# aifoundry-org/MHAQ

Hardware: AMD Instinct MI355X
Metric: qat_images_per_sec (higher is better)
Workload: dtype f32; 1 GPU; ResNet-18 ImageNet-1k QAT step, AEWGS weights per-channel + STE activations, Sym-KL distillation from FP teacher, RAdam, synthetic 224x224, channels_last memory format; per_gpu_batch=250, global_batch=250, parallelism=dp1, sync_batchnorm=False, weight_backward_groups=3, cudnn_benchmark=False

## Files before the change

### include/mhaq_fq.h

```cpp
#ifndef MHAQ_FQ_H
#define MHAQ_FQ_H

#include <stddef.h>
#include <stdint.h>

#ifdef __cplusplus
extern "C" {
#endif

#define MHAQ_FQ_ABI_VERSION 4

enum { MHAQ_FQ_STE = 0, MHAQ_FQ_EWGS = 1, MHAQ_FQ_AEWGS = 2, MHAQ_FQ_LSQ = 3 };

enum {
  MHAQ_FQ_EINVAL = -1,
  MHAQ_FQ_EWORKSPACE = -2,
  MHAQ_FQ_EALIGN = -3,
  MHAQ_FQ_EUNSUPPORTED = -4
};

enum {
  MHAQ_FQ_FLAG_BELOW_MIN = 1,
  MHAQ_FQ_FLAG_ABOVE_MAX = 2,
  MHAQ_FQ_FLAG_NOT_INTEGER = 4
// ... 20 lines not shown
                   void* workspace, size_t workspace_bytes, void* stream);

int mhaq_fq_pt_bwd_partials(const float* x, const float* g, float* gx, int64_t n,
                            const float* s, const float* zp, const float* lo, const float* hi,
                            int method, const float* col_stats, int64_t period,
                            const int8_t* r_sign, uint64_t seed, uint64_t offset, const uint64_t* offset_dev, int count_ties,
                            void* workspace, size_t workspace_bytes, int32_t* nparts_out, void* stream);
int mhaq_fq_pt_bwd_finalize(const void* workspace, int32_t nparts, float* grads , void* stream);

int mhaq_fq_act_fwd(const float* x, float* y, int64_t n,
                    const float* log_act_s, const float* log_act_q, const float* act_b,
                    float* params_out , float* qstats, int32_t* flags,
                    void* workspace, size_t workspace_bytes, void* stream);
size_t mhaq_fq_act_bwd_workspace_bytes(int64_t n);
int mhaq_fq_act_bwd(const float* x, const float* g, float* gx, int64_t n, const float* params ,
                    int method, const int8_t* r_sign, uint64_t seed, uint64_t offset, const uint64_t* offset_dev,
                    float* grads , void* workspace, size_t workspace_bytes, void* stream);

typedef struct {
  const float* partials;
  int64_t nparts;
} mhaq_act_finalize_desc;
int mhaq_fq_act_bwd_partials(const float* x, const float* g, float* gx, int64_t n, const float* params ,
                             int method, const int8_t* r_sign, uint64_t seed, uint64_t offset,
                             const uint64_t* offset_dev, void* workspace, size_t workspace_bytes,
                             int32_t* nparts_out, void* stream);
int mhaq_fq_act_bwd_finalize_multi(const mhaq_act_finalize_desc* descs_device, int nquant,
                                   float* grads_out , void* stream);

enum { MHAQ_FQ_DT_BF16 = 1, MHAQ_FQ_DT_F16 = 2 };
int mhaq_fq_act_fwd_x16(const void* x, void* y, int64_t n, int dtype,
                        const float* log_act_s, const float* log_act_q, const float* act_b,
                        float* params_out , float* qstats, int32_t* flags,
                        void* workspace, size_t workspace_bytes, void* stream);
int mhaq_fq_act_bwd_x16(const void* x, const void* g, void* gx, int64_t n, int dtype, const float* params ,
                        int method, const int8_t* r_sign, uint64_t seed, uint64_t offset, const uint64_t* offset_dev,
                        float* grads , void* workspace, size_t workspace_bytes, void* stream);
int mhaq_fq_act_bwd_partials_x16(const void* x, const void* g, void* gx, int64_t n, int dtype,
                                 const float* params , int method, const int8_t* r_sign, uint64_t seed,
                                 uint64_t offset, const uint64_t* offset_dev, void* workspace, size_t workspace_bytes,
                                 int32_t* nparts_out, void* stream);

int mhaq_fq_act_relu_fwd(const float* z, const float* addend, float* y, float* a_out, int64_t n,
                         const float* log_act_s, const float* log_act_q, const float* act_b,
                         float* params_out , void* stream);
int mhaq_fq_act_relu_bwd(const float* z, const float* g_y, const float* g_a, float* gx, int64_t n,
                         const float* params , int method, uint64_t seed, uint64_t offset,
                         const uint64_t* offset_dev, float* grads , void* workspace, size_t workspace_bytes,
                         void* stream);
int mhaq_fq_act_relu_bwd_partials(const float* z, const float* g_y, const float* g_a, float* gx, int64_t n,
                                  const float* params , int method, uint64_t seed, uint64_t offset,
                                  const uint64_t* offset_dev, void* workspace, size_t workspace_bytes,
                                  int32_t* nparts_out, void* stream);

size_t mhaq_fq_minmax_workspace_bytes(int64_t n);
int mhaq_fq_minmax(const float* x, int64_t n, float* out ,
                   void* workspace, size_t workspace_bytes, void* stream);

int mhaq_fq_row_minmax(const float* w, int64_t co, int64_t row, float* mn_out ,
                       float* mx_out , void* stream);

int mhaq_fq_pt_tie_scatter(const float* w, float* gw, int64_t n, const float* zp,
                           const float* grads , void* stream);

size_t mhaq_fq_pt_aewgs_colstats_workspace_bytes(int64_t co, int64_t row);
int mhaq_fq_pt_aewgs_colstats(const float* w, const float* G, int64_t co, int64_t row,
                              const float* s, const float* zp, const float* lo, const float* hi,
                              float* stats, void* workspace, size_t workspace_bytes, void* stream);

int mhaq_fq_pc_fwd(const float* w, float* wq, float* zp_out , float* q_out ,
                   const float* s , int64_t co, int64_t row, void* stream);

int mhaq_fq_pc_bwd(const float* w, const float* G, float* gw, float* g_s ,
                   const float* s , const float* zp ,
                   int64_t co, int64_t row, int method, const float* stats,
                   const float* gzp_extra ,
                   const int8_t* r_sign, uint64_t seed, uint64_t offset, const uint64_t* offset_dev, void* stream);

int mhaq_fq_wlayer_fwd(const float* w, float* wq, const float* log_s , int64_t co, int64_t row,
                       float* s_out, float* zp_out, float* mx_out, float* lwq_out ,
                       void* stream);
int mhaq_fq_wlayer_bwd(const float* w, const float* G, float* gw, float* g_log_s ,
                       const float* s, const float* zp, const float* mx, const float* g_lwq ,
                       int64_t co, int64_t row, int method, const float* stats,
                       const float* gzp_extra, const int8_t* r_sign, uint64_t seed, uint64_t offset, const uint64_t* offset_dev,
                       void* stream);

int64_t mhaq_fq_wlayer_pt_max_elements(void);
int mhaq_fq_wlayer_pt_fwd(const float* w, float* wq, const float* log_s , int64_t n,
                          float* aux , void* stream);
int mhaq_fq_wlayer_pt_bwd(const float* w, const float* G, float* gw, float* g_log_s ,
                          const float* aux, const float* g_lwq, int64_t n, int method,
                          const int8_t* r_sign, uint64_t seed, uint64_t offset, const uint64_t* offset_dev, void* stream);

size_t mhaq_fq_wlayer_ptl_workspace_bytes(int64_t n);
int mhaq_fq_wlayer_ptl_fwd(const float* w, float* wq, const float* log_s , int64_t n, float* aux ,
                           void* workspace, size_t workspace_bytes, void* stream);
int mhaq_fq_wlayer_ptl_bwd(const float* w, const float* G, float* gw, float* g_log_s ,
                           const float* aux , const float* g_lwq , int64_t n, int method,
                           const float* col_stats, int64_t period,
                           const int8_t* r_sign, uint64_t seed, uint64_t offset, const uint64_t* offset_dev,
                           void* workspace, size_t workspace_bytes, void* stream);

typedef struct {
  const float* w;
  const float* log_s;
// ... 58 lines not shown
```

### mhaq_amd/_lib.py

```python
from __future__ import annotations

import ctypes as C
import os
import re

_HERE = os.path.dirname(os.path.abspath(__file__))
LIB_PATH = os.environ.get("MHAQ_FQ_LIB") or os.path.join(_HERE, "csrc", "libmhaq_fq.so")
HEADER_PATH = os.path.join(os.path.dirname(_HERE), "include", "mhaq_fq.h")

_p = C.c_void_p
_i64 = C.c_int64
_u64 = C.c_uint64
_sz = C.c_size_t
_int = C.c_int

DT_BF16 = 1
DT_F16 = 2

SIGNATURES = {
    "mhaq_fq_abi_version": (_int, []),
    "mhaq_fq_error_string": (C.c_char_p, [_int]),
    "mhaq_fq_fill_r": (_int, [_p, _i64, _u64, _u64, _p]),
    "mhaq_fq_pt_fwd_workspace_bytes": (_sz, [_i64]),
    "mhaq_fq_pt_fwd": (_int, [_p, _p, _i64, _p, _p, _p, _p, _p, _p, _p, _p, _sz, _p]),
    "mhaq_fq_pt_bwd_workspace_bytes": (_sz, [_i64]),
    "mhaq_fq_pt_bwd": (_int, [_p, _p, _p, _i64, _p, _p, _p, _p, _int, _p, _i64, _p, _u64, _u64, _p, _int, _p, _p, _sz, _p]),
    "mhaq_fq_pt_bwd_partials": (_int, [_p, _p, _p, _i64, _p, _p, _p, _p, _int, _p, _i64, _p, _u64, _u64, _p, _int, _p, _sz,
                                       _p, _p]),
    "mhaq_fq_pt_bwd_finalize": (_int, [_p, C.c_int32, _p, _p]),
    "mhaq_fq_act_fwd": (_int, [_p, _p, _i64, _p, _p, _p, _p, _p, _p, _p, _sz, _p]),
    "mhaq_fq_act_bwd_workspace_bytes": (_sz, [_i64]),
    "mhaq_fq_act_bwd": (_int, [_p, _p, _p, _i64, _p, _int, _p, _u64, _u64, _p, _p, _p, _sz, _p]),
    "mhaq_fq_act_bwd_partials": (_int, [_p, _p, _p, _i64, _p, _int, _p, _u64, _u64, _p, _p, _sz, _p, _p]),
    "mhaq_fq_act_bwd_finalize_multi": (_int, [_p, _int, _p, _p]),
    "mhaq_fq_act_fwd_x16": (_int, [_p, _p, _i64, _int, _p, _p, _p, _p, _p, _p, _p, _sz, _p]),
    "mhaq_fq_act_bwd_x16": (_int, [_p, _p, _p, _i64, _int, _p, _int, _p, _u64, _u64, _p, _p, _p, _sz, _p]),
    "mhaq_fq_act_bwd_partials_x16": (_int, [_p, _p, _p, _i64, _int, _p, _int, _p, _u64, _u64, _p, _p, _sz, _p, _p]),
    "mhaq_fq_act_relu_fwd": (_int, [_p, _p, _p, _p, _i64, _p, _p, _p, _p, _p]),
    "mhaq_fq_act_relu_bwd": (_int, [_p, _p, _p, _p, _i64, _p, _int, _u64, _u64, _p, _p, _p, _sz, _p]),
    "mhaq_fq_act_relu_bwd_partials": (_int, [_p, _p, _p, _p, _i64, _p, _int, _u64, _u64, _p, _p, _sz, _p, _p]),
    "mhaq_fq_minmax_workspace_bytes": (_sz, [_i64]),
    "mhaq_fq_minmax": (_int, [_p, _i64, _p, _p, _sz, _p]),
    "mhaq_fq_row_minmax": (_int, [_p, _i64, _i64, _p, _p, _p]),
    "mhaq_fq_pt_tie_scatter": (_int, [_p, _p, _i64, _p, _p, _p]),
    "mhaq_fq_pt_aewgs_colstats_workspace_bytes": (C.c_size_t, [_i64, _i64]),
    "mhaq_fq_pt_aewgs_colstats": (_int, [_p, _p, _i64, _i64, _p, _p, _p, _p, _p, _p, C.c_size_t, _p]),
    "mhaq_fq_pc_fwd": (_int, [_p, _p, _p, _p, _p, _i64, _i64, _p]),
    "mhaq_fq_pc_bwd": (_int, [_p, _p, _p, _p, _p, _p, _i64, _i64, _int, _p, _p, _p, _u64, _u64, _p, _p]),
    "mhaq_fq_pc_aewgs_stats": (_int, [_p, _p, _p, _p, _i64, _i64, _p, _p]),
    "mhaq_fq_wlayer_fwd": (_int, [_p, _p, _p, _i64, _i64, _p, _p, _p, _p, _p]),
    "mhaq_fq_wlayer_bwd": (_int, [_p, _p, _p, _p, _p, _p, _p, _p, _i64, _i64, _int, _p, _p, _p, _u64, _u64, _p, _p]),
    "mhaq_fq_wlayer_fwd_multi": (_int, [_p, _int, _i64, _i64, _p, _p, _p]),
    "mhaq_fq_wlayer_bwd_multi": (_int, [_p, _int, _i64, _i64, _p, _p, _p, _int, _p, _u64, _u64, _p, _p]),
    "mhaq_fq_wlayer_bwd_group": (_int, [_p, _int, _i64, _i64, _p, _i64, _p, _p, _int, _p, _u64, _u64, _p, _p]),
    "mhaq_fq_wlayer_aewgs_stats_group": (_int, [_p, _int, _i64, _p, _i64, _p, _p]),
    "mhaq_fq_pc_quantize": (_int, [_p, _p, _p, _p, _p, _i64, _i64, _p, _p]),
    "mhaq_fq_wlayer_pt_max_elements": (_i64, []),
    "mhaq_fq_wlayer_pt_fwd": (_int, [_p, _p, _p, _i64, _p, _p]),
    "mhaq_fq_wlayer_pt_bwd": (_int, [_p, _p, _p, _p, _p, _p, _i64, _int, _p, _u64, _u64, _p, _p]),
    "mhaq_fq_wlayer_ptl_workspace_bytes": (_sz, [_i64]),
    "mhaq_fq_wlayer_ptl_fwd": (_int, [_p, _p, _p, _i64, _p, _p, _sz, _p]),
    "mhaq_fq_wlayer_ptl_bwd": (_int, [_p, _p, _p, _p, _p, _p, _i64, _int, _p, _i64, _p, _u64, _u64, _p, _p, _sz, _p]),
    "mhaq_fq_vec_fwd": (_int, [_p, _p, _p, _p, _p, _i64, _p]),
    "mhaq_fq_vec_aewgs_stats": (_int, [_p, _p, _p, _p, _i64, _p, _p]),
    "mhaq_fq_vec_bwd": (_int, [_p, _p, _p, _p, _p, _p, _p, _i64, _int, _p, _p, _u64, _u64, _p, _p]),
    "mhaq_fq_potential_loss_fwd": (_int, [_p, _p, _p, _i64, _p, _p, _i64, C.c_float, C.c_float, C.c_float, _int,
                                          _p, _int, _p, _p]),
    "mhaq_fq_potential_loss_bwd": (_int, [_p, _p, _p, _p, _i64, _p, _p, _i64, C.c_float, C.c_float, C.c_float,
                                          _p, _p, _p, _p, _p, _p]),
    "mhaq_fq_noise_fwd": (_int, [_p, _p, _i64, _p]),
    "mhaq_fq_noise_bwd_workspace_bytes": (_sz, [_i64, _i64]),
    "mhaq_fq_noise_bwd": (_int, [_p, _p, _p, _p, _i64, _i64, _int, _p, _i64, _p, _u64, _u64, _p, _p, _sz, _p]),
}

_lib = None


class MhaqFqError(RuntimeError):
    pass


def header_functions():
    with open(HEADER_PATH) as f:
        src = re.sub(r"/\*.*?\*/", "", f.read(), flags=re.S)
    return sorted(set(re.findall(r"\b(mhaq_fq_\w+)\s*\(", src)))


def _try_build() -> None:
    import fcntl
    import subprocess
    import sys
    csrc = os.path.dirname(LIB_PATH)
    with open(os.path.join(csrc, ".build.lock"), "w") as lock:
# ... 37 lines not shown
```

### mhaq_amd/csrc/torch_binding.cpp

```cpp
#include <torch/extension.h>
#include <torch/version.h>
#include <torch/csrc/autograd/custom_function.h>

#include <c10/hip/HIPCachingAllocator.h>
#include <c10/hip/HIPGraphsC10Utils.h>
#include <c10/hip/HIPStream.h>
#include <c10/core/DeviceGuard.h>
#include <dlfcn.h>

#include <algorithm>
#include <atomic>
#include <chrono>
#include <cstring>
#include <map>
#include <memory>
#include <mutex>
#include <string>
#include <unordered_map>
#include <vector>

#include "../../include/mhaq_fq.h"

namespace py = pybind11;
using at::Tensor;
using torch::autograd::AutogradContext;
using torch::autograd::variable_list;

namespace {

#define MHAQ_API(X)                                                                                                   \
  X(mhaq_fq_abi_version) X(mhaq_fq_error_string) X(mhaq_fq_act_fwd) X(mhaq_fq_act_bwd_workspace_bytes)                \
  X(mhaq_fq_act_bwd) X(mhaq_fq_act_bwd_partials) X(mhaq_fq_act_bwd_finalize_multi) X(mhaq_fq_wlayer_fwd)              \
  X(mhaq_fq_wlayer_bwd) X(mhaq_fq_pc_aewgs_stats) X(mhaq_fq_wlayer_fwd_multi) X(mhaq_fq_wlayer_bwd_group)             \
  X(mhaq_fq_wlayer_aewgs_stats_group) X(mhaq_fq_wlayer_pt_fwd) X(mhaq_fq_wlayer_pt_bwd)                               \
  X(mhaq_fq_potential_loss_fwd) X(mhaq_fq_potential_loss_bwd) X(mhaq_fq_wlayer_ptl_workspace_bytes)                   \
  X(mhaq_fq_wlayer_ptl_fwd) X(mhaq_fq_wlayer_ptl_bwd) X(mhaq_fq_pt_aewgs_colstats_workspace_bytes)                     \
  X(mhaq_fq_pt_aewgs_colstats) X(mhaq_fq_act_fwd_x16) X(mhaq_fq_act_bwd_x16) X(mhaq_fq_act_bwd_partials_x16)                    \
  X(mhaq_fq_act_relu_fwd) X(mhaq_fq_act_relu_bwd) X(mhaq_fq_act_relu_bwd_partials)

struct Api {
#define X(n) decltype(&::n) n = nullptr;
  MHAQ_API(X)
#undef X
  void* handle = nullptr;
  std::string path;
};
Api A;

struct MhaqError : std::runtime_error {
  using std::runtime_error::runtime_error;
};

void bind_library(const std::string& path) {
  if (A.handle && A.path == path) return;
  void* h = dlopen(path.c_str(), RTLD_NOW | RTLD_LOCAL);
  if (!h) throw MhaqError("cannot load " + path + ": " + dlerror() + " (there is no CPU fallback)");
  Api a;
#define X(n)                                                                        \
  a.n = reinterpret_cast<decltype(a.n)>(dlsym(h, #n));                              \
  if (!a.n) throw MhaqError(std::string(#n) + " is not exported by " + path);
  MHAQ_API(X)
#undef X
  if (a.mhaq_fq_abi_version() != MHAQ_FQ_ABI_VERSION) throw MhaqError("libmhaq_fq.so ABI version mismatch");
  a.handle = h;
  a.path = path;
  A = a;
}

inline void need_lib() {
  if (!A.handle) throw MhaqError("the C-ABI library is not bound (mhaq_amd._ext.bind)");
}

inline void check(int rc, const char* what) {
  if (rc != 0)
    throw MhaqError(std::string(what) + " failed: " + A.mhaq_fq_error_string(rc) + " (code " + std::to_string(rc) + ")");
}

inline void* cur_stream(const Tensor& t) {
  return (void*)c10::hip::getCurrentHIPStream(t.device().index()).stream();
}

inline bool capturing() {
  return c10::hip::currentStreamCaptureStatusMayInitCtx() != c10::hip::CaptureStatus::None;
}

#define MHAQ_ON_DEVICE_OF(t) const c10::OptionalDeviceGuard mhaq_device_guard_(at::device_of(t))

inline const float* fptr(const Tensor& t) { return static_cast<const float*>(t.const_data_ptr()); }
inline float* fptr_mut(const Tensor& t) { return static_cast<float*>(t.mutable_data_ptr()); }
inline const float* fptr_or_null(const Tensor& t) { return t.defined() ? fptr(t) : nullptr; }

// ... 422 lines not shown
    const int64_t t0 = now_ns();
    auto saved = ctx->get_saved_variables();
    const std::vector<int64_t> ic = ctx->saved_data["i"].toIntVector();
    variable_list out(10);
    const bool g_y_def = grads[0].defined(), g_a_def = ic[4]  != 0 && grads.size() > 2 && grads[2].defined();
    if (!g_y_def && !g_a_def) return out;
    const int64_t t1 = now_ns();
    const size_t e = ic[5] != 0 ? 1 : 0;
    ActGrads res = act_backward(ctx, t0, t1, saved, ic, grads[0], g_a_def ? grads[2] : Tensor(), false,
                                1 + e,
                               [](const ActBwdLaunch& a) {
      if (a.hub)
        check(A.mhaq_fq_act_relu_bwd_partials(fptr(a.x), fptr(a.g), fptr_or_null(a.ga), fptr_mut(a.gx), a.n, fptr(a.params),
                                              a.method, a.d.seed, a.d.offset, a.d.offset_dev, a.ws, a.nb, a.nparts,
                                              a.stream),
              "mhaq_fq_act_relu_bwd_partials");
      else
        check(A.mhaq_fq_act_relu_bwd(fptr(a.x), fptr(a.g), fptr_or_null(a.ga), fptr_mut(a.gx), a.n, fptr(a.params), a.method,
                                     a.d.seed, a.d.offset, a.d.offset_dev, a.gr, a.ws, a.nb, a.stream),
              "mhaq_fq_act_relu_bwd");
    });
    if (e && ctx->needs_input_grad(1)) out[1] = res.gx;
    if (ctx->needs_input_grad(0)) out[0] = std::move(res.gx);
    for (int c = 0; c < 3; ++c) out[2 + c] = std::move(res.gp[c]);
    return out;
  }
};

std::tuple<Tensor, std::optional<Tensor>, Tensor, Tensor, Tensor> act_relu_layer(
    const Tensor& z, const std::optional<Tensor>& addend, const Tensor& log_s, const Tensor& log_q, const Tensor& b,
    int64_t method, bool want_act, int64_t hub_id, int64_t slot, int64_t rank) {
  need_lib();
  MHAQ_ON_DEVICE_OF(z);
  TORCH_CHECK(z.is_cuda() && z.scalar_type() == at::kFloat && z.is_non_overlapping_and_dense(),
              "act_relu_layer: z must be a dense float32 device tensor");
  const bool has_add = addend.has_value() && addend->defined();
  TORCH_CHECK(!has_add || (addend->device() == z.device() && addend->scalar_type() == at::kFloat &&
                           addend->sizes() == z.sizes() && addend->strides() == z.strides()),
              "act_relu_layer: addend must have z's device, dtype, shape and strides");
  TORCH_CHECK(!has_add || want_act, "act_relu_layer: with an addend the ReLU output is an output of the op (want_act)");
  TORCH_CHECK(method == MHAQ_FQ_STE || method == MHAQ_FQ_LSQ || method == MHAQ_FQ_EWGS,
              "act_relu_layer: STE, LSQ or EWGS");
  check_act_params("act_relu_layer", log_s, log_q, b);
  const int64_t t0 = now_ns();
  auto out = ActReluFn::apply(z, addend, log_s, log_q, b, method, want_act, hub_id, slot, rank);
  const Tensor& params = out[1];
  std::tuple<Tensor, std::optional<Tensor>, Tensor, Tensor, Tensor> res{
      out[0], want_act ? std::optional<Tensor>(out[2]) : std::nullopt, params, params.narrow(0, 0, 1),
      params.narrow(0, 3, 1)};
  tick(T_ACT_FWD, t0, now_ns());
  return res;
}

struct Pre {
  bool has = false;
  Tensor wq, s, zp, mx, lwq;
};

PyObject* g_allreduce_avg = nullptr;
std::atomic<bool> g_dist_active{false};

void allreduce_avg(const Tensor& t) {
  py::gil_scoped_acquire gil;
  if (!g_allreduce_avg) throw MhaqError("AEWGS statistics exchange requested but no all-reduce is installed");
  py::reinterpret_borrow<py::object>(g_allreduce_avg)(t);
}

class WeightLayerFn : public torch::autograd::Function<WeightLayerFn> {
 public:
  static variable_list forward(AutogradContext* ctx, const Tensor& w, const Tensor& log_s, int64_t method,
                               const std::optional<Tensor>& r_sign, bool zp_grad, const Pre& pre, int64_t rank,
                               bool distributed) {
    const int64_t co = w.size(0), row = co ? w.numel() / co : 0;
    Tensor wq, s, zp, mx, lwq;
    if (pre.has) {
      wq = pre.wq; s = pre.s; zp = pre.zp; mx = pre.mx; lwq = pre.lwq;
    } else {
      wq = at::empty_like(w);
      Tensor aux = at::empty({4, co}, w.options());
      s = aux.select(0, 0); zp = aux.select(0, 1); mx = aux.select(0, 2); lwq = aux.select(0, 3);
      check(A.mhaq_fq_wlayer_fwd(fptr(w), fptr_mut(wq), fptr(log_s), co, row, fptr_mut(s), fptr_mut(zp), fptr_mut(mx),
                                 fptr_mut(lwq), cur_stream(w)),
            "mhaq_fq_wlayer_fwd");
    }
    weight_save_ctx(ctx, {w, s, zp, mx}, r_sign, method, rank, log_s);
    ctx->saved_data["dist"] = distributed;
    if (!zp_grad) ctx->mark_non_differentiable({s, zp});
    return {wq, zp, s, lwq};
  }

  static variable_list backward(AutogradContext* ctx, variable_list grads) {
    auto saved = ctx->get_saved_variables();
    const Tensor &w = saved[0], &s = saved[1], &zp = saved[2], &mx = saved[3];
    const bool has_r = saved.size() > 4;
    const int64_t method = ctx->saved_data["method"].toInt();
    Tensor G = grads[0].defined() ? like_layout(grads[0], w) : at::zeros_like(w);
    Tensor gzp_extra = grads[1].defined() ? grads[1].contiguous() : Tensor();
    Tensor g_lwq = grads[3].defined() ? grads[3].contiguous() : Tensor();
    const int64_t co = w.size(0), row = co ? w.numel() / co : 0;
    Tensor stats;
    if (method == MHAQ_FQ_AEWGS && ctx->saved_data["dist"].toBool()) {
      stats = at::empty({3, co}, w.options());
      check(A.mhaq_fq_pc_aewgs_stats(fptr(w), fptr(G), fptr(s), fptr(zp), co, row, fptr_mut(stats), cur_stream(w)),
            "mhaq_fq_pc_aewgs_stats");
      allreduce_avg(stats);
    }
// ... 514 lines not shown
    return d;
  }, py::arg("reset") = true);
  m.def("bound_library", []() { return A.path; });

  m.def("rng_manual_seed", [](uint64_t seed) { std::lock_guard<std::mutex> g(R.mu); R.seed = seed; R.seeded = true; R.count = 0; });
  m.def("rng_seed", []() -> py::object { std::lock_guard<std::mutex> g(R.mu); return R.seeded ? py::object(py::int_(R.seed)) : py::none(); });
  m.def("rng_next", [](int64_t rank) {
    std::lock_guard<std::mutex> g(R.mu);
    if (!R.seeded) throw MhaqError("sign stream used before it was seeded");
    return std::make_pair(R.seed ^ ((uint64_t)rank * kGolden), ++R.count);
  });
  m.def("rng_drawn", []() { std::lock_guard<std::mutex> g(R.mu); return R.count; });
  m.def("rng_set_drawn", [](uint64_t n) { std::lock_guard<std::mutex> g(R.mu); R.count = n; });
  m.def("rng_set_base", [](const std::optional<Tensor>& base) {
    std::lock_guard<std::mutex> g(R.mu);
    R.base = (base.has_value() && base->defined()) ? *base : Tensor();
  });
  m.def("rng_base", []() -> std::optional<Tensor> {
    std::lock_guard<std::mutex> g(R.mu);
    return R.base.defined() ? std::optional<Tensor>(R.base) : std::nullopt;
  });

  m.def("set_allreduce_avg", [](py::object fn) {
    g_allreduce_avg = fn.is_none() ? nullptr : fn.inc_ref().ptr();
  });
  m.def("set_dist_active", [](bool v) { g_dist_active.store(v); });

  m.def("hub_create", &hub_create);
  m.def("hub_destroy", [](int64_t id) { g_hubs.erase(id); });
  m.def("hub_begin", &hub_begin);
  m.def("hub_clear_pending", [](int64_t id) { auto h = g_hubs.get(id); std::lock_guard<std::mutex> g(h->mu); h->pending.clear(); });
  m.def("hub_release_captured", [](int64_t id) { g_hubs.get(id)->release_captured(); });
  m.def("hub_state", [](int64_t id) {
    auto h = g_hubs.get(id);
    std::lock_guard<std::mutex> g(h->mu);
    py::dict d;
    d["tables"] = h->tables.entries.size();
    d["captured_tables"] = h->tables.captured();
    d["retired"] = h->retired.size();
    d["pending"] = h->pending.size();
    d["has_table"] = h->last_table.defined();
    int64_t bytes = 0;
    for (auto& w : h->ws) if (w.defined()) bytes += w.numel();
    for (auto& w : h->retired) bytes += w.numel();
    d["workspace_bytes"] = bytes;
    return d;
  });
  m.def("act_layer", &act_layer, py::arg("x"), py::arg("log_act_s"), py::arg("log_act_q"), py::arg("act_b"),
        py::arg("method"), py::arg("r_sign") = py::none(), py::arg("hub") = 0, py::arg("slot") = 0, py::arg("rank") = 0);
  m.def("act_relu_layer", &act_relu_layer, py::arg("z"), py::arg("addend"), py::arg("log_act_s"), py::arg("log_act_q"),
        py::arg("act_b"), py::arg("method"), py::arg("want_act"), py::arg("hub") = 0, py::arg("slot") = 0,
        py::arg("rank") = 0);

  m.def("weight_layer", &weight_layer, py::arg("w"), py::arg("log_wght_s"), py::arg("method"),
        py::arg("r_sign") = py::none(), py::arg("zp_grad") = false, py::arg("pre") = py::none(), py::arg("rank") = 0);
  m.def("weight_layer_pt", &weight_layer_pt, py::arg("w"), py::arg("log_wght_s"), py::arg("method"),
        py::arg("r_sign") = py::none(), py::arg("rank") = 0);
  m.def("weight_layer_ptl", &weight_layer_ptl, py::arg("w"), py::arg("log_wght_s"), py::arg("method"),
        py::arg("r_sign") = py::none(), py::arg("rank") = 0);

  m.def("plan_create", &plan_create);
  m.def("plan_destroy", [](int64_t id) { g_plans.erase(id); });
  m.def("plan_forward", &plan_forward);
  m.def("plan_group_apply", &plan_group_apply);
  m.def("plan_release_captured", [](int64_t id) {
    auto p = g_plans.get(id);
    std::lock_guard<std::mutex> g(p->mu);
    for (auto& grp : p->groups) if (grp.pool) grp.pool->release_captured();
    p->fwd_tables.release_captured();
  });
  m.def("plan_state", [](int64_t id) {
    auto p = g_plans.get(id);
    std::lock_guard<std::mutex> g(p->mu);
    py::dict d;
    d["fwd_tables"] = p->fwd_tables.entries.size();
    py::list pools;
    for (auto& grp : p->groups) {
      py::dict e;
      size_t used = 0, held = 0, size = 0;
      if (grp.pool) {
        size = grp.pool->keys.size();
        for (size_t i = 0; i < size; ++i) { used += grp.pool->used[i]; held += grp.pool->held[i]; }
      }
      e["size"] = size; e["used"] = used; e["held"] = held;
      pools.append(e);
    }
    d["pools"] = pools;
    return d;
  });

  m.def("potential_loss", &potential_loss);
}
```

### mhaq_amd/qat.py

```python
from __future__ import annotations

import contextlib
import copy
import time
from dataclasses import dataclass, field
from typing import Optional

import torch
import torch.distributed as dist
from torch import nn

from . import ops
from ._lib import MhaqFqError
from .enums import QNMethod, QScheme
from .loss import FusedPotentialLoss, FusedPotentialLossNoPred, SymmetricalKL
from .wrap import get_model_values, quantize_model


@dataclass
class QATConfig:
    qscheme: QScheme = QScheme.PER_CHANNEL
    qnmethod: QNMethod = QNMethod.AEWGS
    act_bit: int = 1
    weight_bit: int = 1
    calib_act_bit: int = 10
    calib_weight_bit: int = 10
    excluded_layers: tuple = ("conv1", "fc")
    quantize_bias: bool = False
    distillation: bool = True
    learning_rate: float = 3e-4
    warmup: int = 100
    scale_lr: float = 1.0
    scale_t: float = 2.0
    sync_batchnorm: bool = True
    overlap_teacher: bool = True
    joint_act_finalize: bool = True
    student_high_priority: bool = False
    multi_weight_forward: bool = True
    weight_backward_group_elems: int = 4 << 20
    fuse_blocks: bool = True
    criterion: nn.Module = field(default_factory=nn.CrossEntropyLoss)
    autocast_dtype: Optional[torch.dtype] = None


@torch.no_grad()
def calibrate_weights(model: nn.Module, wbits: int, max_bits: int = 24, row_minmax_fn=None) -> None:
    row_minmax_fn = row_minmax_fn or ops.row_minmax
    for m in model.modules():
        if hasattr(m, "log_wght_s") and hasattr(m, "weight"):
            mn, mx = row_minmax_fn(m.weight)
            mn, mx = mn.cpu(), mx.cpu()
            if m.log_wght_s.numel() == 1 and mn.numel() != 1:
                mn, mx = mn.min(), mx.max()
            if not m.log_wght_s.requires_grad:
                wbits = max_bits
            floor = torch.log2((mx - mn) / (2 ** wbits - 1)).reshape(m.log_wght_s.shape)
            m.log_wght_s.copy_(torch.max(m.log_wght_s.detach().cpu(), floor))


def _cpu_row_minmax(w):
    dims = tuple(range(1, w.dim()))
    return w.detach().amin(dims), w.detach().amax(dims)


@torch.no_grad()
def calibrate_activations(model: nn.Module, batches, abits: int, max_bits: int = 24, minmax_fn=None) -> None:
    minmax_fn = minmax_fn or ops.minmax
    acts = [m for m in model.modules() if hasattr(m, "log_act_s") and hasattr(m, "act_b")]
    seen = {id(a): [] for a in acts}
    hooks = [a.register_forward_pre_hook(lambda mod, inp: seen[id(mod)].append(minmax_fn(inp[0]))) for a in acts]
    was_training = model.training
    model.eval()
    for x in batches:
        model(x)
    for h in hooks:
        h.remove()
    model.train(was_training)
    for a in acts:
        mm = torch.stack(seen[id(a)]).cpu()
        mn, mx = mm[:, 0].min(), mm[:, 1].max()
        if not a.log_act_q.requires_grad and not a.log_act_s.requires_grad:
            abits = max_bits
        if mx - mn > 0:
            log_s = torch.log2((mx - mn) / (2 ** abits - 1))
            a.act_b.fill_(mn)
            a.log_act_s.fill_(log_s)
            a.log_act_q.fill_(log_s + abits)
        else:
            a.log_act_q.zero_(), a.log_act_s.zero_(), a.act_b.fill_(mn)
            a.log_act_q.requires_grad_(False), a.log_act_s.requires_grad_(False), a.act_b.requires_grad_(False)


class TemperatureSchedule:
# ... 23 lines not shown
        new_lr = self.lr * self.lr_t if past else self.lr * self.total_batch / self.warmup
        self._set_lr(optimizer, new_lr)
        return new_lr


class _QATModule(nn.Module):

    def __init__(self, net, qscheme, act_hub=None, weight_forward=None):
        super().__init__()
        self.model = net
        self.qscheme = qscheme
        self.act_hub = act_hub
        self.weight_forward = weight_forward
        self._quantized = None

    def forward(self, x):
        if self.weight_forward is not None and self.training:
            self.weight_forward.run()
        if self.act_hub is not None and self.training:
            self.act_hub.begin()
        if self._quantized is None:
            self._quantized = [m for m in self.model.modules() if hasattr(m, "log_wght_s") or hasattr(m, "log_act_s")]
        try:
            return (self.model(x), *get_model_values(self.model, self.qscheme, modules=self._quantized))
        finally:
            if self.act_hub is not None:
                self.act_hub.end()


class QATTrainer:
    def __init__(self, net: nn.Module, cfg: QATConfig, device, calib_batches=None, layers=None,
                 distributed=None, minmax_fn=None, optimizer_factory=None,
                 multi_tensor_weights=False, capture_graph=None, loss_classes=None):
        self.cfg, self.device = cfg, torch.device(device)
        if cfg.autocast_dtype is not None and cfg.autocast_dtype != torch.bfloat16:
            raise ValueError(f"QATConfig.autocast_dtype: {cfg.autocast_dtype} is not supported (None or torch.bfloat16; "
                             "float16 training needs loss scaling, which this trainer does not do)")
        self.distributed = ops._dist_active() if distributed is None else distributed
        net = net.to(self.device)
        self.teacher = copy.deepcopy(net).eval().requires_grad_(False) if cfg.distillation else None
        quantize_model(net, cfg.qscheme, cfg.qnmethod, cfg.excluded_layers, cfg.quantize_bias, cfg.act_bit,
                       layers=layers)
        net.to(self.device)
        if calib_batches is not None:
            calibrate_weights(net, cfg.calib_weight_bit,
                              row_minmax_fn=_cpu_row_minmax if self.device.type != "cuda" else None)
            calibrate_activations(net, calib_batches, cfg.calib_act_bit, minmax_fn=minmax_fn)
        if self.distributed and cfg.sync_batchnorm and self.device.type == "cuda":
            net = nn.SyncBatchNorm.convert_sync_batchnorm(net)
        if cfg.fuse_blocks and layers is None and self.device.type == "cuda":
            from . import fused_blocks
            if fused_blocks.enabled_by_env():
                fused_blocks.install(net)
        self.net = net
        self.teacher_stream = None
        if cfg.distillation and cfg.overlap_teacher and self.device.type == "cuda":
            self.teacher_stream = torch.cuda.Stream(device=self.device)
        self._hp_stream = None
        if cfg.student_high_priority and self.device.type == "cuda":
            self._hp_stream = torch.cuda.Stream(device=self.device, priority=-1)
        self.multi = None
        if multi_tensor_weights and self.distributed:
            raise ValueError("multi_tensor_weights is a single-GPU option (the data-parallel trainer keeps the "
                             "per-layer ops: AEWGS statistics all-reduce + gradient overlap)")
        if multi_tensor_weights:
            from .multi import MultiTensorWeightQuant
            self.multi = MultiTensorWeightQuant(net)
        self.act_hub = None
        if cfg.joint_act_finalize and self.device.type == "cuda" and (layers is None):
            from .act_hub import ActGradHub
            hub = ActGradHub(net)
            self.act_hub = hub if len(hub) > 1 else None
        self.weight_forward = None
        if cfg.multi_weight_forward and self.multi is None and self.device.type == "cuda" and layers is None:
            from .multi import MultiTensorWeightQuant
            try:
                wf = MultiTensorWeightQuant(net, joint_backward=False,
                                            backward_group_elems=cfg.weight_backward_group_elems)
                self.weight_forward = wf if wf.nlayers > 1 else None
            except ValueError:
                pass
        self.module = _QATModule(net, cfg.qscheme, self.act_hub, self.weight_forward)
        self._flat_sync = False
        want_capture = capture_graph
        if want_capture is None:
            want_capture = "auto" if (layers is None and optimizer_factory is None and not multi_tensor_weights) else False
        if self.distributed and want_capture and self.device.type == "cuda" and self.multi is None:
            step_collectives = any(isinstance(m, nn.SyncBatchNorm) for m in net.modules()) or any(
                ops._method_value(m.Q.qnmethod) == QNMethod.AEWGS.value for m in net.modules() if hasattr(m, "Q")
            ) or next(iter(net.buffers()), None) is not None
            self._flat_sync = not step_collectives
        if self.distributed:
            for p in [m.log_b_s for m in net.modules() if hasattr(m, "log_b_s")]:
                p.requires_grad_(False)
            if self._flat_sync:
                with torch.no_grad():
                    for t in list(net.parameters()) + list(net.buffers()):
                        dist.broadcast(t, 0)
            else:
                self._wrap_ddp()
        if loss_classes is None:
            if self.device.type != "cuda":
                raise MhaqFqError("QATTrainer on a CPU device needs loss_classes (and layers): the fake-quant path and "
                                  "its PotentialLoss run only as HIP kernels (no CPU fallback by design)")
            loss_classes = (FusedPotentialLoss, FusedPotentialLossNoPred)
        if cfg.distillation:
# ... 279 lines not shown
```

Before: 6119 images/s.

## Add custom HIP BatchNorm backward kernels for channels-last fp32 student BN layers

Swaps the student's nn.BatchNorm2d modules for a subclass whose autograd node keeps the framework forward but runs a custom HIP backward. The backward does a chunked fp64 per-channel reduction, a finalize kernel that writes dweight/dbias and per-channel constants, and a vectorized dx kernel with non-temporal loads and stores for large tensors. The aim is to replace MIOpen/PyTorch BN backward on channels-last fp32 inputs. It costs three launches per BN plus a workspace allocation, and it falls back to the stock backward when the inputs are not eligible.

```diff
diff --git a/include/mhaq_fq.h b/include/mhaq_fq.h
--- a/include/mhaq_fq.h
+++ b/include/mhaq_fq.h
@@ -96,6 +96,11 @@
                                   const float* params , int method, uint64_t seed, uint64_t offset,
                                   const uint64_t* offset_dev, void* workspace, size_t workspace_bytes,
                                   int32_t* nparts_out, void* stream);
+
+size_t mhaq_fq_bn_bwd_workspace_bytes(int64_t m, int64_t c);
+int mhaq_fq_bn_bwd(const float* x, const float* dy, const float* mean, const float* invstd, const float* weight,
+                   float* dx, float* dweight, float* dbias, int64_t m, int64_t c,
+                   void* workspace, size_t workspace_bytes, void* stream);
 
 size_t mhaq_fq_minmax_workspace_bytes(int64_t n);
 int mhaq_fq_minmax(const float* x, int64_t n, float* out ,
diff --git a/mhaq_amd/_lib.py b/mhaq_amd/_lib.py
--- a/mhaq_amd/_lib.py
+++ b/mhaq_amd/_lib.py
@@ -39,6 +39,8 @@
     "mhaq_fq_act_relu_fwd": (_int, [_p, _p, _p, _p, _i64, _p, _p, _p, _p, _p]),
     "mhaq_fq_act_relu_bwd": (_int, [_p, _p, _p, _p, _i64, _p, _int, _u64, _u64, _p, _p, _p, _sz, _p]),
     "mhaq_fq_act_relu_bwd_partials": (_int, [_p, _p, _p, _p, _i64, _p, _int, _u64, _u64, _p, _p, _sz, _p, _p]),
+    "mhaq_fq_bn_bwd_workspace_bytes": (_sz, [_i64, _i64]),
+    "mhaq_fq_bn_bwd": (_int, [_p, _p, _p, _p, _p, _p, _p, _p, _i64, _i64, _p, _sz, _p]),
     "mhaq_fq_minmax_workspace_bytes": (_sz, [_i64]),
     "mhaq_fq_minmax": (_int, [_p, _i64, _p, _p, _sz, _p]),
     "mhaq_fq_row_minmax": (_int, [_p, _i64, _i64, _p, _p, _p]),
diff --git a/mhaq_amd/bn_backward.py b/mhaq_amd/bn_backward.py
--- /dev/null
+++ b/mhaq_amd/bn_backward.py
@@ -0,0 +1,46 @@
+from __future__ import annotations
+
+import os
+
+import torch
+from torch import nn
+
+ENV_SWITCH = "MHAQ_BN_BACKWARD"
+
+
+def enabled_by_env() -> bool:
+    return os.environ.get(ENV_SWITCH, "1").strip().lower() not in ("0", "false", "off", "no")
+
+
+class HipBackwardBatchNorm2d(nn.BatchNorm2d):
+
+    def forward(self, input):
+        if (not self.training or not self.track_running_stats or not self.affine or not input.is_cuda
+                or input.dtype != torch.float32 or self.weight.dtype != torch.float32):
+            return super().forward(input)
+        self._check_input_dim(input)
+        exponential_average_factor = 0.0 if self.momentum is None else self.momentum
+        if self.num_batches_tracked is not None:
+            self.num_batches_tracked.add_(1)
+            if self.momentum is None:
+                exponential_average_factor = 1.0 / float(self.num_batches_tracked)
+            else:
+                exponential_average_factor = self.momentum
+        from . import _ext
+        return _ext.ext().bn_train(input, self.weight, self.bias, self.running_mean, self.running_var,
+                                   exponential_average_factor, self.eps, torch.backends.cudnn.enabled)
+
+
+def install(model: nn.Module) -> int:
+    switched = 0
+    for m in model.modules():
+        if type(m) is nn.BatchNorm2d:
+            m.__class__ = HipBackwardBatchNorm2d
+            switched += 1
+    return switched
+
+
+def uninstall(model: nn.Module) -> None:
+    for m in model.modules():
+        if type(m) is HipBackwardBatchNorm2d:
+            m.__class__ = nn.BatchNorm2d
diff --git a/mhaq_amd/csrc/bn_bwd.hip b/mhaq_amd/csrc/bn_bwd.hip
--- /dev/null
+++ b/mhaq_amd/csrc/bn_bwd.hip
@@ -0,0 +1,236 @@
+#include "fq_common.hpp"
+
+namespace mhaq {
+
+template <bool NT>
+__device__ __forceinline__ vf4 bn_ld4(const float* p, int64_t vidx) {
+  const vf4* q = reinterpret_cast<const vf4*>(p) + vidx;
+  return NT ? __builtin_nontemporal_load(q) : *q;
+}
+__device__ __forceinline__ void bn_st4(float* p, int64_t vidx, vf4 v) {
+  __builtin_nontemporal_store(v, reinterpret_cast<vf4*>(p) + vidx);
+}
+
+constexpr int kBnCols = 16;
+constexpr int kBnRedU = 4;
+constexpr int kBnMinRows = 448;
+constexpr int kBnMaxChunks = 2048;
+constexpr int kBnDxU = 2;
+constexpr int64_t kBnMaxChannels = 1ll << 22;
+constexpr int kBnNConst = 5;
+
+struct BnGeom {
+  int64_t rows;
+  int64_t nchunks;
+  int ncol;
+};
+static inline BnGeom bn_geom(int64_t m, int64_t c) {
+  const int64_t cv = c >> 2;
+  const int64_t cols = cv < kBnCols ? cv : kBnCols;
+  const int64_t rpp = kBlock / cols;
+  const int64_t unit = rpp * kBnRedU;
+  int64_t rows = (m + kBnMaxChunks - 1) / kBnMaxChunks;
+  if (rows < kBnMinRows) rows = kBnMinRows;
+  rows = (rows + unit - 1) / unit * unit;
+  BnGeom g;
+  g.rows = rows;
+  g.nchunks = (m + rows - 1) / rows;
+  g.ncol = (int)((cv + kBnCols - 1) / kBnCols);
+  return g;
+}
+
+constexpr int64_t kBnReduceNtElems = 28ll << 20;
+constexpr int64_t kBnDxNtElems = 28ll << 20;
+constexpr int64_t kBnBigElems = 20ll << 20;
+constexpr int kBnMinWaves = 8, kBnBigMaxWaves = 6;
+
+template <bool NT>
+__global__ __launch_bounds__(kBlock) void bn_bwd_reduce_kernel(
+    const float* __restrict__ x, const float* __restrict__ dy, const float* __restrict__ mean,
+    double* __restrict__ partials, int64_t m, int cv, int64_t rows) {
+  const int c0 = (int)blockIdx.y * kBnCols;
+  const int cols = (cv - c0) < kBnCols ? (cv - c0) : kBnCols;
+  const int rpp = kBlock / cols;
+  const int ty = (int)(threadIdx.x / (uint32_t)cols), tx = (int)threadIdx.x - ty * cols;
+  const bool live = ty < rpp;
+  const int64_t row0 = (int64_t)blockIdx.x * rows;
+  const int64_t rend = (row0 + rows < m) ? row0 + rows : m;
+  const int64_t colv = c0 + tx;
+  float mu[4];
+#pragma unroll
+  for (int j = 0; j < 4; ++j) mu[j] = mean[colv * 4 + j];
+  double s1[4] = {0, 0, 0, 0}, s2[4] = {0, 0, 0, 0};
+  for (int64_t rb = row0 + ty; rb - ty < rend; rb += (int64_t)rpp * kBnRedU) {
+    vf4 a[kBnRedU], b[kBnRedU];
+    bool ok[kBnRedU];
+#pragma unroll
+    for (int u = 0; u < kBnRedU; ++u) {
+      const int64_t r = rb + (int64_t)u * rpp;
+      ok[u] = live && r < rend;
+      const int64_t vidx = (ok[u] ? r : rend - 1) * cv + colv;
+      a[u] = bn_ld4<NT>(x, vidx);
+      b[u] = bn_ld4<NT>(dy, vidx);
+    }
+    __builtin_amdgcn_sched_barrier(0);
+#pragma unroll
+    for (int u = 0; u < kBnRedU; ++u) {
+      const float av[4] = {a[u].x, a[u].y, a[u].z, a[u].w}, bv[4] = {b[u].x, b[u].y, b[u].z, b[u].w};
+#pragma unroll
+      for (int j = 0; j < 4; ++j) {
+        const double g = ok[u] ? (double)bv[j] : 0.0;
+        const double d = ok[u] ? (double)av[j] - (double)mu[j] : 0.0;
+        s1[j] += g;
+        s2[j] = fma(g, d, s2[j]);
+      }
+    }
+  }
+  __shared__ __align__(16) double sm[kBlock * 8];
+  const int w = 4 * cols;
+  if (live) {
+#pragma unroll
+    for (int j = 0; j < 4; ++j) {
+      sm[(ty * 2 + 0) * w + tx * 4 + j] = s1[j];
+      sm[(ty * 2 + 1) * w + tx * 4 + j] = s2[j];
+    }
+  }
+  __syncthreads();
+  if ((int)threadIdx.x < 2 * w) {
+    const int k = (int)threadIdx.x >= w ? 1 : 0, c = (int)threadIdx.x - k * w;
+    double tot = 0.0;
+    for (int r = 0; r < rpp; ++r) tot += sm[(r * 2 + k) * w + c];
+    partials[((int64_t)blockIdx.x * 2 + k) * ((int64_t)cv * 4) + (int64_t)c0 * 4 + c] = tot;
+  }
+}
+
+__global__ __launch_bounds__(kBlock) void bn_bwd_finalize_kernel(
+    const double* __restrict__ partials, int nchunks, int c, const float* __restrict__ mean,
+    const float* __restrict__ invstd, const float* __restrict__ weight, double inv_m, float* __restrict__ consts,
+    float* __restrict__ dweight, float* __restrict__ dbias) {
+  const int ch = (int)blockIdx.x * 4;
+  double v[8] = {0, 0, 0, 0, 0, 0, 0, 0};
+  for (int i = threadIdx.x; i < nchunks; i += kBlock) {
+    const double* p0 = partials + ((int64_t)i * 2 + 0) * c + ch;
+    const double* p1 = partials + ((int64_t)i * 2 + 1) * c + ch;
+#pragma unroll
+    for (int j = 0; j < 4; ++j) {
+      v[j] += p0[j];
+      v[4 + j] += p1[j];
+    }
+  }
+  __shared__ double sm[8 * (kBlock / 64)];
+  block_sum<8>(v, sm);
+  if (threadIdx.x == 0) {
+#pragma unroll
+    for (int j = 0; j < 4; ++j) {
+      const float is = invstd[ch + j], g = weight ? weight[ch + j] : 1.0f;
+      const double db = v[j], dw = (double)is * v[4 + j];
+      consts[0 * c + ch + j] = mean[ch + j];
+      consts[1 * c + ch + j] = is;
+      consts[2 * c + ch + j] = g * is;
+      consts[3 * c + ch + j] = (float)(db * inv_m);
+      consts[4 * c + ch + j] = (float)(dw * inv_m);
+      if (dweight) dweight[ch + j] = (float)dw;
+      if (dbias) dbias[ch + j] = (float)db;
+    }
+  }
+}
+
+template <bool NT, bool BIG>
+__global__ __attribute__((amdgpu_waves_per_eu((BIG ? 1 : kBnMinWaves), (BIG ? kBnBigMaxWaves : kBnMinWaves))))
+__launch_bounds__(kBlock) void bn_bwd_dx_kernel(
+    const float* __restrict__ x, const float* __restrict__ dy, float* __restrict__ dx, int64_t nvec, int cv,
+    const float* __restrict__ consts) {
+  const int64_t blk0 = (int64_t)blockIdx.x * (kBlock * kBnDxU);
+  const int64_t base = blk0 + threadIdx.x;
+  const bool full = blk0 + kBlock * kBnDxU <= nvec;
+  vf4 a[kBnDxU], b[kBnDxU];
+#pragma unroll
+  for (int u = 0; u < kBnDxU; ++u) {
+    const int64_t idx = base + u * kBlock;
+    const int64_t idc = (full || idx < nvec) ? idx : nvec - 1;
+    a[u] = bn_ld4<NT>(x, idc);
+    b[u] = bn_ld4<NT>(dy, idc);
+  }
+  __builtin_amdgcn_sched_barrier(0);
+  const uint32_t ucv = (uint32_t)cv;
+  const uint32_t cb = ((blockIdx.x % ucv) * ((uint32_t)(kBlock * kBnDxU) % ucv)) % ucv;
+  const uint32_t step = (uint32_t)kBlock % ucv;
+  uint32_t col = (cb + threadIdx.x) % ucv;
+  const int64_t c = (int64_t)cv * 4;
+  float k[kBnNConst][4];
+#pragma unroll
+  for (int u = 0; u < kBnDxU; ++u) {
+    const int64_t idx = base + u * kBlock;
+    if (u > 0) {
+      col += step;
+      if (col >= ucv) col -= ucv;
+    }
+    if (u == 0 || step != 0) {
+#pragma unroll
+      for (int q = 0; q < kBnNConst; ++q) ldv<4>(consts + q * c + (int64_t)col * 4, k[q]);
+    }
+    if (full || idx < nvec) {
+      const float xv[4] = {a[u].x, a[u].y, a[u].z, a[u].w}, gv[4] = {b[u].x, b[u].y, b[u].z, b[u].w};
+      float o[4];
+#pragma unroll
+      for (int j = 0; j < 4; ++j) {
+        const float xh = (xv[j] - k[0][j]) * k[1][j];
+        o[j] = k[2][j] * ((gv[j] - k[3][j]) - xh * k[4][j]);
+      }
+      bn_st4(dx, idx, vf4{o[0], o[1], o[2], o[3]});
+    }
+  }
+}
+
+static inline bool bn_aligned(const void* p, uintptr_t a) { return ((uintptr_t)p & (a - 1)) == 0; }
+
+}
+
+using namespace mhaq;
+
+extern "C" {
+
+size_t mhaq_fq_bn_bwd_workspace_bytes(int64_t m, int64_t c) {
+  if (m <= 0 || c <= 0 || (c & 3) || c > kBnMaxChannels) return 0;
+  return ((size_t)kBnNConst * sizeof(float) + 2 * (size_t)bn_geom(m, c).nchunks * sizeof(double)) * (size_t)c;
+}
+
+int mhaq_fq_bn_bwd(const float* x, const float* dy, const float* mean, const float* invstd, const float* weight,
+                   float* dx, float* dweight, float* dbias, int64_t m, int64_t c, void* workspace,
+                   size_t workspace_bytes, void* stream) {
+  if (m <= 0 || c <= 0 || !x || !dy || !mean || !invstd || !workspace) return MHAQ_FQ_EINVAL;
+  if ((c & 3) || c > kBnMaxChannels || m > (INT64_MAX >> 3) / c) return MHAQ_FQ_EUNSUPPORTED;
+  if (workspace_bytes < mhaq_fq_bn_bwd_workspace_bytes(m, c)) return MHAQ_FQ_EWORKSPACE;
+  if (!bn_aligned(x, 16) || !bn_aligned(dy, 16) || !bn_aligned(dx, 16) || !bn_aligned(workspace, 16) ||
+      !bn_aligned(mean, 4) || !bn_aligned(invstd, 4) || !bn_aligned(weight, 4) || !bn_aligned(dweight, 4) ||
+      !bn_aligned(dbias, 4))
+    return MHAQ_FQ_EALIGN;
+  const BnGeom g = bn_geom(m, c);
+  const int64_t nvec = m * (c >> 2);
+  const int64_t dx_grid = (nvec + kBlock * kBnDxU - 1) / (kBlock * kBnDxU);
+  if (g.nchunks > 0x7fffffff || dx_grid > 0x7fffffff) return MHAQ_FQ_EUNSUPPORTED;
+  if (!dx && !dweight && !dbias) return 0;
+  hipStream_t st = (hipStream_t)stream;
+  float* consts = (float*)workspace;
+  double* parts = (double*)(consts + kBnNConst * c);
+  const int cv = (int)(c >> 2);
+  const bool nt_r = m * c >= kBnReduceNtElems, nt_d = m * c >= kBnDxNtElems, big = m * c >= kBnBigElems;
+  const dim3 rgrid((unsigned)g.nchunks, (unsigned)g.ncol);
+  if (nt_r) MHAQ_LAUNCH(bn_bwd_reduce_kernel<true>, rgrid, dim3(kBlock), 0, st, x, dy, mean, parts, m, cv, g.rows);
+  else MHAQ_LAUNCH(bn_bwd_reduce_kernel<false>, rgrid, dim3(kBlock), 0, st, x, dy, mean, parts, m, cv, g.rows);
+  int rc = launch_status();
+  if (rc) return rc;
+  MHAQ_LAUNCH(bn_bwd_finalize_kernel, dim3((unsigned)cv), dim3(kBlock), 0, st, (const double*)parts, (int)g.nchunks,
+              (int)c, mean, invstd, weight, 1.0 / (double)m, consts, dweight, dbias);
+  rc = launch_status();
+  if (rc || !dx) return rc;
+  const dim3 dgrid((unsigned)dx_grid);
+#define MHAQ_LAUNCH_BN_DX(NT, BG) \
+  MHAQ_LAUNCH((bn_bwd_dx_kernel<NT, BG>), dgrid, dim3(kBlock), 0, st, x, dy, dx, nvec, cv, (const float*)consts)
+  if (big) { if (nt_d) MHAQ_LAUNCH_BN_DX(true, true); else MHAQ_LAUNCH_BN_DX(false, true); }
+  else { if (nt_d) MHAQ_LAUNCH_BN_DX(true, false); else MHAQ_LAUNCH_BN_DX(false, false); }
+#undef MHAQ_LAUNCH_BN_DX
+  return launch_status();
+}
+
+}
diff --git a/mhaq_amd/csrc/torch_binding.cpp b/mhaq_amd/csrc/torch_binding.cpp
--- a/mhaq_amd/csrc/torch_binding.cpp
+++ b/mhaq_amd/csrc/torch_binding.cpp
@@ -36,7 +36,8 @@
   X(mhaq_fq_potential_loss_fwd) X(mhaq_fq_potential_loss_bwd) X(mhaq_fq_wlayer_ptl_workspace_bytes)                   \
   X(mhaq_fq_wlayer_ptl_fwd) X(mhaq_fq_wlayer_ptl_bwd) X(mhaq_fq_pt_aewgs_colstats_workspace_bytes)                     \
   X(mhaq_fq_pt_aewgs_colstats) X(mhaq_fq_act_fwd_x16) X(mhaq_fq_act_bwd_x16) X(mhaq_fq_act_bwd_partials_x16)                    \
-  X(mhaq_fq_act_relu_fwd) X(mhaq_fq_act_relu_bwd) X(mhaq_fq_act_relu_bwd_partials)
+  X(mhaq_fq_act_relu_fwd) X(mhaq_fq_act_relu_bwd) X(mhaq_fq_act_relu_bwd_partials)                                    \
+  X(mhaq_fq_bn_bwd_workspace_bytes) X(mhaq_fq_bn_bwd)
 
 struct Api {
 #define X(n) decltype(&::n) n = nullptr;
@@ -565,6 +566,88 @@
   return res;
 }
 
+inline bool aligned16(const Tensor& t) { return (reinterpret_cast<uintptr_t>(t.const_data_ptr()) & 15) == 0; }
+
+inline bool bn_bwd_eligible(const Tensor& x, const Tensor& w, const Tensor& mean, const Tensor& invstd) {
+  if (!x.is_cuda() || x.scalar_type() != at::kFloat || x.dim() != 4 || x.numel() == 0) return false;
+  if (!x.is_contiguous(at::MemoryFormat::ChannelsLast) || (x.size(1) & 3) || !aligned16(x)) return false;
+  auto stat_ok = [&](const Tensor& t) {
+    return t.defined() && t.is_cuda() && t.scalar_type() == at::kFloat && t.is_contiguous() && t.numel() == x.size(1);
+  };
+  return stat_ok(mean) && stat_ok(invstd) && (!w.defined() || stat_ok(w));
+}
+
+std::atomic<int64_t> g_bn_hip_backwards{0};
+
+class BatchNormTrainFn : public torch::autograd::Function<BatchNormTrainFn> {
+ public:
+  static Tensor forward(AutogradContext* ctx, const Tensor& x, const std::optional<Tensor>& w,
+                        const std::optional<Tensor>& b, const std::optional<Tensor>& running_mean,
+                        const std::optional<Tensor>& running_var, double momentum, double eps, bool cudnn_enabled) {
+    auto out = at::_batch_norm_impl_index(x, w, b, running_mean, running_var, true, momentum, eps,
+                                          cudnn_enabled);
+    const bool has_w = w.has_value() && w->defined();
+    ctx->save_for_backward({x, has_w ? *w : Tensor(), std::get<1>(out), std::get<2>(out), std::get<3>(out)});
+    ctx->saved_data["impl"] = std::get<4>(out);
+    ctx->saved_data["eps"] = eps;
+    if (running_mean.has_value() && running_mean->defined()) ctx->saved_data["rm"] = *running_mean;
+    if (running_var.has_value() && running_var->defined()) ctx->saved_data["rv"] = *running_var;
+    ctx->set_materialize_grads(false);
+    return std::get<0>(out);
+  }
+
+  static variable_list backward(AutogradContext* ctx, variable_list grads) {
+    variable_list out(8);
+    if (!grads[0].defined()) return out;
+    TORCH_CHECK(!(at::GradMode::is_enabled() && grads[0].requires_grad()),
+                "bn_train: the node is once-differentiable (no double backward)");
+    at::NoGradGuard no_grad;
+    auto saved = ctx->get_saved_variables();
+    const Tensor &x = saved[0], &w = saved[1], &mean = saved[2], &invstd = saved[3], &reserve = saved[4];
+    const std::array<bool, 3> mask = {ctx->needs_input_grad(0), w.defined() && ctx->needs_input_grad(1),
+                                      ctx->needs_input_grad(2)};
+    if (!bn_bwd_eligible(x, w, mean, invstd)) {
+      auto opt = [](const Tensor& t) { return t.defined() ? std::optional<Tensor>(t) : std::nullopt; };
+      auto get = [&](const char* k) {
+        return ctx->saved_data.count(k) ? std::optional<Tensor>(ctx->saved_data[k].toTensor()) : std::nullopt;
+      };
+      auto g = at::_batch_norm_impl_index_backward(ctx->saved_data["impl"].toInt(), x, grads[0], opt(w), get("rm"),
+                                                   get("rv"), opt(mean), opt(invstd), true,
+                                                   ctx->saved_data["eps"].toDouble(), mask, reserve);
+      if (mask[0]) out[0] = std::get<0>(g);
+      if (mask[1]) out[1] = std::get<1>(g);
+      if (mask[2]) out[2] = std::get<2>(g);
+      return out;
+    }
+    need_lib();
+    const int64_t c = x.size(1), m = x.numel() / c;
+    const Tensor dy = like_layout(grads[0].scalar_type() == at::kFloat ? grads[0] : grads[0].to(at::kFloat), x);
+    Tensor dx = mask[0] ? at::empty_like(x) : Tensor();
+    Tensor dw = mask[1] ? at::empty_like(w) : Tensor();
+    Tensor db = mask[2] ? at::empty({c}, mean.options()) : Tensor();
+    const size_t nb = A.mhaq_fq_bn_bwd_workspace_bytes(m, c);
+    Tensor ws = at::empty({(int64_t)nb}, x.options().dtype(at::kByte));
+    check(A.mhaq_fq_bn_bwd(fptr(x), fptr(dy), fptr(mean), fptr(invstd), fptr_or_null(w), mask[0] ? fptr_mut(dx) : nullptr,
+                           mask[1] ? fptr_mut(dw) : nullptr, mask[2] ? fptr_mut(db) : nullptr, m, c, ws.mutable_data_ptr(),
+                           nb, cur_stream(x)),
+          "mhaq_fq_bn_bwd");
+    g_bn_hip_backwards.fetch_add(1, std::memory_order_relaxed);
+    out[0] = dx;
+    out[1] = dw;
+    out[2] = db;
+    return out;
+  }
+};
+
+Tensor bn_train(const Tensor& x, const std::optional<Tensor>& w, const std::optional<Tensor>& b,
+                const std::optional<Tensor>& running_mean, const std::optional<Tensor>& running_var, double momentum,
+                double eps, bool cudnn_enabled) {
+  TORCH_CHECK(w.has_value() && w->defined() && b.has_value() && b->defined(),
+              "bn_train: an affine BatchNorm (weight and bias) is required");
+  MHAQ_ON_DEVICE_OF(x);
+  return BatchNormTrainFn::apply(x, w, b, running_mean, running_var, momentum, eps, cudnn_enabled);
+}
+
 struct Pre {
   bool has = false;
   Tensor wq, s, zp, mx, lwq;
@@ -1185,6 +1268,12 @@
         py::arg("act_b"), py::arg("method"), py::arg("want_act"), py::arg("hub") = 0, py::arg("slot") = 0,
         py::arg("rank") = 0);
 
+  m.def("bn_train", &bn_train, py::arg("x"), py::arg("weight"), py::arg("bias"), py::arg("running_mean"),
+        py::arg("running_var"), py::arg("momentum"), py::arg("eps"), py::arg("cudnn_enabled") = true);
+
+  m.def("bn_hip_backwards", []() { return g_bn_hip_backwards.load(); },
+        "number of BatchNorm backwards so far that ran the HIP kernels instead of the framework's backward");
+
   m.def("weight_layer", &weight_layer, py::arg("w"), py::arg("log_wght_s"), py::arg("method"),
         py::arg("r_sign") = py::none(), py::arg("zp_grad") = false, py::arg("pre") = py::none(), py::arg("rank") = 0);
   m.def("weight_layer_pt", &weight_layer_pt, py::arg("w"), py::arg("log_wght_s"), py::arg("method"),
diff --git a/mhaq_amd/qat.py b/mhaq_amd/qat.py
--- a/mhaq_amd/qat.py
+++ b/mhaq_amd/qat.py
@@ -39,6 +39,7 @@
     multi_weight_forward: bool = True
     weight_backward_group_elems: int = 4 << 20
     fuse_blocks: bool = True
+    hip_bn_backward: bool = True
     criterion: nn.Module = field(default_factory=nn.CrossEntropyLoss)
     autocast_dtype: Optional[torch.dtype] = None
 
@@ -168,6 +169,10 @@
             from . import fused_blocks
             if fused_blocks.enabled_by_env():
                 fused_blocks.install(net)
+        if cfg.hip_bn_backward and layers is None and self.device.type == "cuda":
+            from . import bn_backward
+            if bn_backward.enabled_by_env():
+                bn_backward.install(net)
         self.net = net
         self.teacher_stream = None
         if cfg.distillation and cfg.overlap_teacher and self.device.type == "cuda":
```

After: 6428 images/s (median of 6 runs). +5.0%, better.
